# parsaeskandar/pangenome-index

Measured on AMD Instinct MI355X. Metric: find_mems reads/sec (150 bp batch), higher is better.
Workload: dtype u64

## Files before the change

### pangenome-index_amd/csrc/pgx_batch.hip

```cpp
#include <memory>
#include <string>
#include <thread>

#include "pgx_runtime_internal.hpp"

struct pgx_chunk { uint64_t r0, r1, slot_base, slots; };

struct pgx_batch {
    pgx_index *h = nullptr;
    pgx_device_image *dimg = nullptr;
    int device = 0;
    hipStream_t own = nullptr;
    hipStream_t side = nullptr;
    hipEvent_t ev_side[2] = {nullptr, nullptr};
    bool class_valid = false, class_ok = false;
    uint64_t side_reads_est = 0;
    uint64_t n_reads = 0, read_bytes = 0;
    HostBuf h_off[2];
    int h_off_cur = 0;
    const uint64_t *h_offsets() const { return h_off[h_off_cur].as<uint64_t>(); }
    std::vector<pgx_chunk> chunks;
    bool plan_valid = false, slot_off_valid = false;
    uint64_t slot_off_min_len = 0;
    uint64_t plan_min_len = 0, plan_budget = 0;
// ... 292 lines not shown
    PGX_GUARD_END
}

extern "C" pgx_status pgx_batch_upload_text(pgx_batch *b, const uint8_t *text, uint64_t n_bytes, uint32_t format, uint64_t *n_reads) {
    PGX_GUARD_BEGIN
    RoctxRange range("pgx_batch_upload_text");
    if (!b || !n_reads || (!text && n_bytes)) throw Error(PGX_ERR_ARG, "pgx_batch_upload_text: null argument");
    if (format > PGX_READS_FASTQ) throw Error(PGX_ERR_ARG, "pgx_batch_upload_text: unknown format " + std::to_string(format));
    use_device(b->device);
    batch_upload_text(b, text, n_bytes, format, n_reads);
    return PGX_OK;
    PGX_GUARD_END
}


struct RunKnobs {
    bool spec;
    bool arena;
    bool has_arena_cap;
    uint64_t arena_cap;
    uint64_t budget_slots;
    bool narrow;
    bool force_redo;
    bool pairs;
    bool side;
    bool packed;
    int coop;
    bool lce;
    bool has_wg_per_cu;
    int wg_per_cu;
    uint32_t heavy_ext;
    bool has_side_heavy_ext;
    uint32_t side_heavy_ext;
    bool debug_counters;
    bool fm_stats;
};

static RunKnobs read_run_knobs() {
    auto is_set = [](const char *name) { return std::getenv(name) != nullptr; };
    auto not_zero = [](const char *name) { const char *e = std::getenv(name); return !(e && e[0] == '0'); };
    RunKnobs k{};
    k.spec = not_zero("PGX_SPEC");
    k.arena = not_zero("PGX_SLOT_ARENA");
    if (const char *e = std::getenv("PGX_SLOT_ARENA_CAP")) { k.has_arena_cap = true; k.arena_cap = std::strtoull(e, nullptr, 10); }
    if (const char *e = std::getenv("PGX_SLOT_BUDGET_MB")) k.budget_slots = std::max<uint64_t>(1, std::strtoull(e, nullptr, 10)) * (1ull << 20) / sizeof(pgx_mem);
    k.narrow = not_zero("PGX_FM_NARROW");
    k.force_redo = is_set("PGX_FM_NARROW_FORCE_REDO");
    k.pairs = not_zero("PGX_FM_PAIRS");
    k.side = !is_set("PGX_FM_NO_SIDE");
    k.packed = not_zero("PGX_FM_PACKED");
    k.coop = -1;
    if (const char *e = std::getenv("PGX_FM_COOP")) k.coop = e[0] == '1';
    k.lce = not_zero("PGX_FM_LCE");
    if (const char *e = std::getenv("PGX_FM_WG_PER_CU")) { k.has_wg_per_cu = true; k.wg_per_cu = std::atoi(e); }
    k.heavy_ext = PGX_FM_HEAVY_EXT;
    if (const char *e = std::getenv("PGX_FM_HEAVY_EXT")) k.heavy_ext = (uint32_t)std::strtoul(e, nullptr, 10);
    if (const char *e = std::getenv("PGX_FM_SIDE_HEAVY_EXT")) { k.has_side_heavy_ext = true; k.side_heavy_ext = (uint32_t)std::strtoul(e, nullptr, 10); }
    k.debug_counters = is_set("PGX_DEBUG_COUNTERS");
    k.fm_stats = is_set("PGX_FM_STATS");
    return k;
}

static const void *find_mems_entry(bool in_lds, uint32_t kind, bool narrow, bool seeded) {
    using K = const void *;
    static const K tab[2][4][2][2] = {
        {{{(K)pgx_find_mems_kernel<false, 0, false, false>, nullptr}, {nullptr, nullptr}},
         {{(K)pgx_find_mems_kernel<false, 1, false, false>, (K)pgx_find_mems_kernel<false, 1, false, true>},
          {(K)pgx_find_mems_kernel<false, 1, true, false>, (K)pgx_find_mems_kernel<false, 1, true, true>}},
         {{(K)pgx_find_mems_kernel<false, 2, false, false>, (K)pgx_find_mems_kernel<false, 2, false, true>},
          {(K)pgx_find_mems_kernel<false, 2, true, false>, (K)pgx_find_mems_kernel<false, 2, true, true>}},
         {{(K)pgx_find_mems_kernel<false, 3, false, false>, (K)pgx_find_mems_kernel<false, 3, false, true>}, {nullptr, nullptr}}},
        {{{(K)pgx_find_mems_kernel<true, 0, false, false>, nullptr}, {nullptr, nullptr}},
         {{(K)pgx_find_mems_kernel<true, 1, false, false>, (K)pgx_find_mems_kernel<true, 1, false, true>},
          {(K)pgx_find_mems_kernel<true, 1, true, false>, (K)pgx_find_mems_kernel<true, 1, true, true>}},
         {{nullptr, nullptr}, {nullptr, nullptr}},
         {{nullptr, nullptr}, {nullptr, nullptr}}}};
    return kind < 4 ? tab[in_lds][kind][narrow][seeded] : nullptr;
}

static uint32_t find_mems_bits(bool in_lds, uint32_t kind, bool narrow, bool seeded) {
    return PGX_KERNELS_FM | (seeded ? PGX_KERNELS_FM_SEEDED : 0u) | (narrow ? PGX_KERNELS_FM_NARROW : 0u) | (kind << PGX_KERNELS_FM_KIND_SHIFT) | (in_lds ? PGX_KERNELS_FM_LDS : 0u);
}

static const void *find_mems_variant(bool in_lds, uint32_t kind, bool narrow, bool seeded, uint32_t &bits) {
    if (kind == 0) seeded = false;
    const void *f = find_mems_entry(in_lds, kind, narrow, seeded);
    if (!f) throw Error(PGX_ERR_UNSUPPORTED, "pgx_batch_run: no find_mems kernel for this image");
    bits = find_mems_bits(in_lds, kind, narrow, seeded);
    return f;
}
// ... 12 lines not shown
    if (lce) return (wide || !packed || coop) ? nullptr : with_lce[s64];
    if (!packed) return coop ? nullptr : plain[wide][s64];
    return pack[wide][coop][s64];
}

static uint32_t find_mems_pairs_bits(bool wide, bool packed, bool coop, bool s64, bool lce) {
    return PGX_KERNELS_PAIRS | (s64 ? PGX_KERNELS_PAIRS_S64 : 0u) | (coop ? PGX_KERNELS_PAIRS_COOP : 0u) | (packed ? PGX_KERNELS_PAIRS_PACKED : 0u) |
           (wide ? PGX_KERNELS_PAIRS_WIDE : 0u) | (lce ? PGX_KERNELS_PAIRS_LCE : 0u);
}

static const void *find_mems_pairs_variant(bool wide, bool packed, bool coop, bool s64, bool lce, uint32_t &bits) {
    const void *f = find_mems_pairs_entry(wide, packed, coop, s64, lce);
    if (!f && lce) throw Error(PGX_ERR_UNSUPPORTED, "pgx_batch_run: no LCE pairs kernel for this image");
    if (!f) throw Error(PGX_ERR_UNSUPPORTED, "pgx_batch_run: no cooperative pairs kernel without the packed reads");
    bits = find_mems_pairs_bits(wide, packed, coop, s64, lce);
    return f;
}

extern "C" uint32_t pgx_kernel_variants(uint32_t *out, uint32_t cap) {
    uint32_t n = 0;
    auto put = [&](uint32_t bits) { if (out && n < cap) out[n] = bits; n++; };
    for (int c = 0; c < 32; c++) {
        const bool in_lds = c & 16, narrow = c & 2, seeded = c & 1;
        const uint32_t kind = (c >> 2) & 3;
        if (find_mems_entry(in_lds, kind, narrow, seeded)) put(find_mems_bits(in_lds, kind, narrow, seeded));
    }
    for (int c = 0; c < 32; c++) {
        const bool wide = c & 16, packed = c & 8, coop = c & 4, s64 = c & 2, lce = c & 1;
        if (find_mems_pairs_entry(wide, packed, coop, s64, lce)) put(find_mems_pairs_bits(wide, packed, coop, s64, lce));
    }
    return n;
}

struct RunCtx {
    pgx_batch *b;
    hipStream_t s;
    RunKnobs k;
    PgxDevImage img;
    uint64_t n, min_len, min_occ;
    bool want_tags;
    unsigned long long *ctr = nullptr;
    bool spec = false, arena_on = false;
    uint64_t cm_cap = 0;
    const void *kfn = nullptr, *kfn_wide = nullptr, *kfn_pairs = nullptr;
    uint32_t kfn_bits = 0, kfn_pairs_bits = 0;
    size_t pairs_lds = 0;
    int cus = 0;
    bool fresh_work = false, fresh_mark = false;
    uint64_t n_ext = 0;
    float ms_fm = 0, ms_cp = 0, ms_main = 0;
};

struct FmArgs {
    PgxDevImage img;
    const uint8_t *reads;
    const uint64_t *off, *slot_off;
    uint64_t n, min_len, min_occ, base, first;
    pgx_mem *slots;
    uint32_t *cnt;
    unsigned long long *next, *cur;
    uint32_t hext, hcap;
    pgx_heavy_item *hlist;
    unsigned long long *hcount;
    uint32_t *ovf;
    uint64_t ovf_cap;
};

static void record(pgx_batch *b, int i, hipStream_t s) {
    static const char *const stage[10] = {"pgx: run begins (classify, sizing)", "pgx: find_mems launches follow", "pgx: find_mems enqueued", "pgx: compaction enqueued",
                                          "pgx: tag locate enqueued", "pgx: tag gather enqueued", "pgx: tag sort/unique enqueued", "pgx: run enqueued", "pgx: main find_mems kernel enqueued",
                                          "pgx: per-upload passes enqueued"};
    if (roctx().on) roctx().mark(stage[i]);
    if (!b->timed) return;
    if (!b->ev[i]) HIPCHECK(hipEventCreate(&b->ev[i]));
    HIPCHECK(hipEventRecord(b->ev[i], s));
}

static unsigned find_mems_grid(const RunCtx &r, const void *kfn, size_t lds, bool few_suffice, uint64_t cn) {
    int wg = 0;
    HIPCHECK(hipOccupancyMaxActiveBlocksPerMultiprocessor(&wg, kfn, PGX_FM_THREADS, lds));
// ... 62 lines not shown

static void classify_reads(RunCtx &r, uint64_t cn) {
    pgx_batch *b = r.b;
    hipStream_t s = r.s;
    r.fresh_work = true;
    const uint64_t cap = std::max<uint64_t>(cn, 1024);
    b->read_flags.ensure(((cn + 3) & ~3ull) + 4);
    b->side_list.ensure((cn ? cn : 1) * sizeof(pgx_heavy_item));
    b->side_count.ensure(16);
    b->scan_tmp.ensure(cap * 8);
    b->scan_tmp.scan_epoch = 0;
    b->packed.ensure(((b->read_bytes + 15) / 16 + 64) * 4);
    HIPCHECK(hipMemsetAsync(b->side_count.p, 0, 16, s));
    HIPCHECK(hipMemsetAsync(b->read_flags.p, 0, ((cn + 3) & ~3ull) + 4, s));
    unsigned long long *d_bad = b->side_count.as<unsigned long long>() + 1;
    hipLaunchKernelGGL(pgx_bad_chunks_kernel, dim3(std::min<unsigned>(grid_for((b->read_bytes + 15) / 16, 256), (unsigned)r.cus * 16u)), dim3(256), 0, s,
                       (const uint8_t *)b->reads.as<uint8_t>(), b->read_bytes, b->scan_tmp.as<uint64_t>(), d_bad, cap, b->packed.as<uint32_t>());
    HIPCHECK(hipGetLastError());
    unsigned long long n_bad = 0;
    read_scalars(&n_bad, d_bad, sizeof n_bad, s);
    b->class_ok = n_bad <= cap;
    b->side_reads_est = n_bad / 4;
    if (b->class_ok && n_bad) {
        hipLaunchKernelGGL(pgx_classify_reads_kernel, dim3(grid_for(n_bad, 256)), dim3(256), 0, s, (const uint8_t *)b->reads.as<uint8_t>(),
                           (const uint64_t *)b->offsets.as<uint64_t>(), cn, (const uint64_t *)b->scan_tmp.as<uint64_t>(), (const unsigned long long *)d_bad, cap,
                           b->read_flags.as<uint32_t>(), b->side_list.as<pgx_heavy_item>(), b->side_count.as<unsigned long long>());
        HIPCHECK(hipGetLastError());
    }
    b->class_valid = true;
}

static void launch_side(RunCtx &r, FmArgs &a, const void *kf, unsigned grid) {
    pgx_batch *b = r.b;
    HIPCHECK(hipEventRecord(b->ev_side[0], r.s));
    HIPCHECK(hipStreamWaitEvent(b->side, b->ev_side[0], 0));
    const pgx_heavy_item *s_list = b->side_list.as<pgx_heavy_item>();
    const unsigned long long *s_count = b->side_count.as<unsigned long long>();
    unsigned long long *s_cur = r.ctr + PGX_CTR_SIDE_CURSOR;
    uint32_t s_hext = r.k.heavy_ext ? std::min<uint32_t>(r.k.heavy_ext, PGX_FM_SIDE_HEAVY_EXT) : 0u;
    if (r.k.has_side_heavy_ext) s_hext = r.k.side_heavy_ext;
    void *sargs[] = {&a.img, &a.reads, &a.off, &a.n, &a.min_len, &a.min_occ, &a.slot_off, &a.slots, &a.cnt, &a.next, &s_cur, &a.first, &a.base,
                     &s_hext, &a.hcap, &a.hlist, &a.hcount, &s_list, &s_count, &a.ovf, &a.ovf_cap};
    const uint64_t cus = (uint64_t)r.cus;
    const unsigned side_wgs = (unsigned)std::min<uint64_t>(4 * cus, std::max<uint64_t>(cus, b->side_reads_est / (2ull * PGX_FM_THREADS) + 1));
    HIPCHECK(hipLaunchKernel(kf, dim3(std::min<unsigned>(grid, side_wgs)), dim3(PGX_FM_THREADS), sargs, b->dimg->lds_bytes, b->side));
    b->timing.kernels |= r.kfn_bits | PGX_KERNELS_SIDE | (kf != r.kfn ? PGX_KERNELS_FM_REDO : 0u);
    HIPCHECK(hipEventRecord(b->ev_side[1], b->side));
}

static void launch_pairs(RunCtx &r, FmArgs &a, const uint8_t *skip, uint64_t cn, unsigned grid) {
    pgx_batch *b = r.b;
    const PgxDevImage &img = r.img;
    const void *kp = r.kfn_pairs;
    uint32_t kp_bits = r.kfn_pairs_bits;
    size_t plds = r.pairs_lds;
    const uint32_t *a_packed = nullptr;
    uint32_t a_pkw = 0;
    const uint32_t pkw = (uint32_t)((15 + b->max_read_len + 15) >> 4) + 1u;
    if (skip && pkw <= 24 && r.k.packed) {
        const bool coop = r.k.coop >= 0 ? r.k.coop != 0 : b->h->img.pairs.size() > (3ull << 30);
        const bool lce = img.lce_sa && !coop && !img.wide && r.min_occ <= 1 && r.k.lce;
        kp = find_mems_pairs_variant(img.wide != 0, true, coop, img.pairs_stride == PGX_PAIRS_STRIDE64, lce, kp_bits);
        const size_t lce_lds = lce ? (size_t)PGX_FM_THREADS * (16 + 4 + 20) : 0;
        a_packed = b->packed.as<uint32_t>();
        a_pkw = pkw;
        plds = (size_t)pkw * PGX_FM_THREADS * 4 + (coop ? (size_t)(PGX_FM_THREADS / 64) * 8192 : 0) + (img.wide ? (size_t)img.n_sbp * 192 : 0) + lce_lds;
        b->timing.pairs_reads = lce ? 4u : coop ? 3u : 2u;
        grid = find_mems_grid(r, kp, plds, true, cn);
    }
    void *pargs[] = {&a.img, &a.reads, &a.off, &a.n, &a.min_len, &a.min_occ, &a.slot_off, &a.slots, &a.cnt, &a.next, &a.cur, &a.first, &a.base,
                     &a.hext, &a.hcap, &a.hlist, &a.hcount, &skip, &a_packed, &a_pkw, &a.ovf, &a.ovf_cap};
    HIPCHECK(hipLaunchKernel(kp, dim3(grid), dim3(PGX_FM_THREADS), pargs, plds, r.s));
    b->timing.kernels |= kp_bits;
}

static uint64_t arena_slots(const RunCtx &r, const pgx_chunk &c) {
    const pgx_batch *b = r.b;
    if (!r.arena_on) return 0;
    const uint64_t cn = c.r1 - c.r0;
    uint64_t want = b->shape_valid && b->shape_reads == r.n && b->shape_min_len == r.min_len && b->chunks.size() == 1 ? with_slack(b->last_ovf_used) + 4096 : 8 * cn + 4096;
    if (r.k.has_arena_cap) want = r.k.arena_cap;
    want = std::max<uint64_t>(want, b->max_read_len + 1);
    want = std::max<uint64_t>(want, (uint64_t)PGX_ARENA_SUBS * (b->max_read_len + 1));
    want = (want + PGX_ARENA_SUBS - 1) / PGX_ARENA_SUBS * PGX_ARENA_SUBS;
    return want < c.slots && want < (1ull << 32) ? want : 0;
}

static uint64_t find_mems_chunk(RunCtx &r, size_t ci, uint64_t &ovf_cap) {
    pgx_batch *b = r.b;
    hipStream_t s = r.s;
    const pgx_chunk &c = b->chunks[ci];
    const uint64_t cn = c.r1 - c.r0;
    const bool one_chunk = b->chunks.size() == 1;
    const uint32_t heavy_ext = r.k.heavy_ext;
    const unsigned grid = find_mems_grid(r, r.kfn_pairs ? r.kfn_pairs : r.kfn, r.kfn_pairs ? r.pairs_lds : b->dimg->lds_bytes, r.img.dense != 0, cn);
    uint64_t *local = b->mem_off.as<uint64_t>() + c.r0;
    const void *kf = r.kfn;
    ovf_cap = arena_slots(r, c);
    for (int attempt = 0;; attempt++) {
        b->slots.ensure(((ovf_cap ? ovf_cap : c.slots) + 4 * cn) * sizeof(pgx_mem));
        if (ci || attempt) {
            HIPCHECK(hipMemsetAsync(r.ctr, 0, PGX_CTR_TAG0 * 8, s));
            HIPCHECK(hipMemsetAsync(r.ctr + PGX_CTR_ARENA0, 0, (PGX_CTR_ALL - PGX_CTR_ARENA0) * 8, s));
        }
        FmArgs a;
        a.img = r.img;
        a.reads = b->reads.as<uint8_t>();
        a.off = b->offsets.as<uint64_t>(); a.slot_off = b->slot_off.as<uint64_t>();
        a.n = c.r1; a.min_len = r.min_len; a.min_occ = r.min_occ; a.base = c.slot_base; a.first = c.r0;
        a.slots = b->slots.as<pgx_mem>();
        a.cnt = b->mem_count.as<uint32_t>();
        a.next = r.ctr; a.cur = r.ctr + PGX_CTR_CURSOR;
        a.hext = heavy_ext; a.hcap = PGX_FM_HEAVY_CAP;
        a.hlist = b->heavy_list.as<pgx_heavy_item>();
        a.hcount = r.ctr + PGX_CTR_HEAVY;
        a.ovf = b->ovf_base.as<uint32_t>() - c.r0;
        a.ovf_cap = ovf_cap;
        bool side_running = false;
        if (r.kfn_pairs) {
            const uint8_t *skip = nullptr;
            if (one_chunk && r.k.side) {
                if (!b->side) {
                    HIPCHECK(hipStreamCreateWithFlags(&b->side, hipStreamNonBlocking));
                    for (auto &e : b->ev_side) HIPCHECK(hipEventCreateWithFlags(&e, hipEventDisableTiming));
                }
                if (!b->class_valid) classify_reads(r, cn);
                record(b, 9, s); r.fresh_mark = true;
                if (b->class_ok) {
                    skip = b->read_flags.as<uint8_t>();
                    launch_side(r, a, kf, grid);
                    side_running = true;
                }
            }
            launch_pairs(r, a, skip, cn, grid);
        } else {
            const pgx_heavy_item *a_rlist = nullptr;
            const unsigned long long *a_rcount = nullptr;
            void *args[] = {&a.img, &a.reads, &a.off, &a.n, &a.min_len, &a.min_occ, &a.slot_off, &a.slots, &a.cnt, &a.next, &a.cur, &a.first, &a.base,
                            &a.hext, &a.hcap, &a.hlist, &a.hcount, &a_rlist, &a_rcount, &a.ovf, &a.ovf_cap};
            if (ci == 0 && attempt == 0) { record(b, 9, s); r.fresh_mark = true; }
            HIPCHECK(hipLaunchKernel(kf, dim3(grid), dim3(PGX_FM_THREADS), args, b->dimg->lds_bytes, s));
            b->timing.kernels |= r.kfn_bits | (kf != r.kfn ? PGX_KERNELS_FM_REDO : 0u);
        }
        record(b, 8, s);
        if (side_running) HIPCHECK(hipStreamWaitEvent(s, b->ev_side[1], 0));
        if (heavy_ext) {
            b->timing.kernels |= PGX_KERNELS_HEAVY;
            if (b->dimg->lds_bytes)
                hipLaunchKernelGGL(pgx_find_mems_heavy_kernel<true>, dim3(PGX_FM_HEAVY_GRID), dim3(256), b->dimg->lds_bytes, s, r.img, a.reads, a.off,
                                   r.min_len, r.min_occ, a.slot_off, c.slot_base, a.slots, a.cnt, r.ctr, (const pgx_heavy_item *)a.hlist,
                                   (const unsigned long long *)a.hcount, (uint32_t)PGX_FM_HEAVY_CAP, b->heavy_scratch.as<PgxHeavyResult>(), c.r0, cn, a.ovf, a.ovf_cap);
            else
                hipLaunchKernelGGL(pgx_find_mems_heavy_kernel<false>, dim3(PGX_FM_HEAVY_GRID), dim3(256), 0, s, r.img, a.reads, a.off, r.min_len, r.min_occ,
                                   a.slot_off, c.slot_base, a.slots, a.cnt, r.ctr, (const pgx_heavy_item *)a.hlist,
                                   (const unsigned long long *)a.hcount, (uint32_t)PGX_FM_HEAVY_CAP, b->heavy_scratch.as<PgxHeavyResult>(), c.r0, cn, a.ovf, a.ovf_cap);
        }
        if (ovf_cap) hipLaunchKernelGGL(pgx_arena_demand_kernel, dim3(1), dim3(PGX_ARENA_SUBS), 0, s, r.ctr);
        HIPCHECK(hipGetLastError());
        b->timing.find_mems_launches++;
        record(b, 2, s);
        scan_excl(0, b->mem_count.as<uint32_t>() + c.r0, cn, 0, local, b->scan_tmp, s, reinterpret_cast<uint64_t *>(r.ctr + PGX_CTR_MEMS));
        if (r.spec) return r.cm_cap;
        unsigned long long cc[16];
        read_scalars(cc, r.ctr, sizeof cc, s);
        if (ovf_cap) b->last_ovf_used = cc[PGX_CTR_OVF_TOP];
        if (ovf_cap && cc[PGX_CTR_OVF_ABORT]) { ovf_cap = 0; continue; }
        const bool forced = attempt == 0 && kf != r.kfn_wide && r.k.force_redo;
        if ((cc[PGX_CTR_OVF32] || forced) && kf != r.kfn_wide) { kf = r.kfn_wide; continue; }
        r.n_ext += cc[PGX_CTR_EXT];
        b->timing.heavy_reads += (uint32_t)std::min<unsigned long long>(cc[PGX_CTR_HEAVY], PGX_FM_HEAVY_CAP);
        b->timing.pairs_other_steps += (uint32_t)cc[PGX_CTR_REDO];
        return cc[PGX_CTR_MEMS];
    }
}

static void compact_chunk(RunCtx &r, const pgx_chunk &c, uint64_t cm, uint64_t mem_base, uint64_t ovf_cap) {
    pgx_batch *b = r.b;
    hipStream_t s = r.s;
    const uint64_t cn = c.r1 - c.r0;
    b->mems.ensure_keep((mem_base + cm ? mem_base + cm : 1) * sizeof(pgx_mem), mem_base * sizeof(pgx_mem));
    hipLaunchKernelGGL(pgx_compact_mems_kernel, dim3(grid_for(cn, 256)), dim3(256), 0, s, c.r0, cn, b->slot_off.as<uint64_t>(),
                       c.slot_base, b->slots.as<pgx_mem>(), b->mem_count.as<uint32_t>(), (const uint64_t *)(b->mem_off.as<uint64_t>() + c.r0), mem_base,
                       b->mems.as<pgx_mem>(), r.spec ? r.cm_cap : ~0ull, reinterpret_cast<uint64_t *>(r.ctr + PGX_CTR_ABORT),
                       (const uint32_t *)(b->ovf_base.as<uint32_t>() - c.r0), ovf_cap);
    HIPCHECK(hipGetLastError());
    record(b, 3, s);
    if (b->timed && b->chunks.size() > 1) {
        HIPCHECK(hipStreamSynchronize(s));
// ... 62 lines not shown
        if (r.want_tags) {
            b->timing.ms_tag_locate = el(3, 4);
            b->timing.ms_tag_gather = el(4, 5);
            b->timing.ms_tag_sort = el(5, 6);
        }
        b->timing.ms_total = el(0, 7);
        if (r.fresh_work) b->timing.ms_per_upload = b->ms_upload_passes + (r.fresh_mark ? el(0, 9) : 0.0f);
    }
    if (r.fresh_work) b->ms_upload_passes = 0;
    return true;
}

static bool run_pass(RunCtx &r, bool may_speculate, bool &force_worst) {
    pgx_batch *b = r.b;
    hipStream_t s = r.s;
    b->n_mems = b->n_positions = b->n_ext = b->n_tag_overflow = 0;
    std::memset(&b->timing, 0, sizeof b->timing);
    r.fresh_work = r.fresh_mark = false;
    r.n_ext = 0;
    r.ms_fm = r.ms_cp = r.ms_main = 0;
    b->counters.ensure(PGX_CTR_ALL * 8);
    HIPCHECK(hipMemsetAsync(b->counters.p, 0, PGX_CTR_ALL * 8, s));
    r.ctr = b->counters.as<unsigned long long>();

    record(b, 0, s);
    plan_slots(r);
    const std::vector<pgx_chunk> &chunks = b->chunks;
    r.arena_on = r.k.arena && !force_worst;
    r.kfn = r.kfn_wide = r.kfn_pairs = nullptr;
    r.cus = 0;
    if (r.n) choose_kernels(r);
    if (r.k.heavy_ext) {
        b->heavy_list.ensure((size_t)PGX_FM_HEAVY_CAP * sizeof(pgx_heavy_item));
        b->heavy_scratch.ensure((size_t)PGX_FM_HEAVY_GRID * PGX_FM_HEAVY_MAXLEN * sizeof(PgxHeavyResult));
    }
    r.spec = may_speculate && chunks.size() == 1 && b->shape_valid && b->shape_reads == r.n && b->shape_min_len == r.min_len && b->shape_min_occ == r.min_occ &&
             b->shape_tags == r.want_tags && (!r.want_tags || (b->tw.have_last && b->tw.last_largest <= PGX_SORT_WG_LDS_CAP)) && r.k.spec && !r.k.force_redo;
    r.cm_cap = with_slack(b->last_mems);
    uint64_t mem_base = 0;
    for (size_t ci = 0; ci < chunks.size(); ci++) {
        record(b, 1, s);
        uint64_t ovf_cap = 0;
        const uint64_t cm = find_mems_chunk(r, ci, ovf_cap);
        compact_chunk(r, chunks[ci], cm, mem_base, ovf_cap);
        mem_base += cm;
    }
    b->n_mems = mem_base;
    if (!r.kfn_pairs) b->timing.pairs_reads = 0u;
    else if (!b->timing.pairs_reads) b->timing.pairs_reads = 1u;
    b->timing.seed_depth = (r.img.seed_k != 0 && r.min_len >= r.img.seed_k && r.img.dense) ? r.img.seed_k : 0u;
    if (chunks.size() != 1) {
        if (chunks.empty()) { record(b, 1, s); record(b, 2, s); }
        scan_excl(0, b->mem_count.p, r.n, 0, b->mem_off.as<uint64_t>(), b->scan_tmp, s);
        b->mems.ensure_keep((b->n_mems ? b->n_mems : 1) * sizeof(pgx_mem), b->n_mems * sizeof(pgx_mem));
        record(b, 3, s);
    }
    record(b, 3, s);
    if (r.want_tags) {
        tag_pipeline(r.img, b->mems.as<pgx_mem>(), nullptr, nullptr, b->n_mems, b->tw, r.ctr + PGX_CTR_TAG_OVERFLOW, r.ctr + PGX_CTR_TAG0, s,
                     [&](int stage) { record(b, 4 + stage, s); }, r.spec, reinterpret_cast<const uint64_t *>(r.ctr + PGX_CTR_MEMS),
                     reinterpret_cast<uint64_t *>(r.ctr + PGX_CTR_ABORT));
        b->n_positions = b->tw.n_positions;
        b->ran_tags = true;
    }
    record(b, 7, s);
    return read_back(r, force_worst);
}
// ... 379 lines not shown
```

### pangenome-index_amd/csrc/pgx_device.h

```cpp
#pragma once

#include <hip/hip_runtime.h>
#include <stdint.h>

#include "../../include/pgx.h"
#include "pgx_image.h"

enum PgxCounterSlot {
    PGX_CTR_EXT = 0,
    PGX_CTR_TAG_OVERFLOW = 1,
    PGX_CTR_CURSOR = 5,
    PGX_CTR_HEAVY = 8,
    PGX_CTR_OVF32 = 9,
    PGX_CTR_MEMS = 10,
    PGX_CTR_REDO = 11,
    PGX_CTR_REDO_CURSOR = 12,
    PGX_CTR_SIDE_CURSOR = 13,
    PGX_CTR_OVF_TOP = 14,
    PGX_CTR_OVF_ABORT = 15,
    PGX_CTR_TAG0 = 16,
    PGX_CTR_ABORT = 30,
    PGX_CTR_PAIRS_LINES = 32,
    PGX_CTR_PAIRS_SEEDS = 33,
    PGX_CTR_FM_LINES = 34,
// ... 43 lines not shown
    const uint4 *seed_main, *seed_small;
    const uint4 *pairs;
    const uint4 *first_ext;
    uint32_t pair_runs;
    const uint64_t *sbase2, *pbase;
    uint32_t d2_sb_shift, pairs_sb_shift, n_sb2, n_sbp;
    uint32_t wide;
    uint32_t pairs_stride;
    const uint32_t *lce_sa;
    const uint32_t *lce_text;
    const uint32_t *lce_flags;
    const uint8_t *lce_lcp;
    uint32_t lce_max;
    uint32_t refill_min;
};
#define PGX_LCP_CAP 254u
#define PGX_LCP_UNKNOWN 255u
#define PGX_SEED_UNUSABLE 255u
#define PGX_SEED_MAX_K 16
#define PGX_SEED_SMALL_K 10

struct pgx_heavy_item {
    uint64_t rid;
    uint32_t x, nm;
};
struct PgxHeavyResult {
    pgx_mem mem;
    uint32_t next_x, n_ext, has_mem, pad;
};
#define PGX_FM_HEAVY_EXT 2048u
#define PGX_FM_SIDE_HEAVY_EXT 2048u
#define PGX_FM_HEAVY_MAXLEN 4096u
#define PGX_FM_HEAVY_CAP 8192u
#define PGX_FM_HEAVY_GRID 64u

template <bool LDS_IMAGE, int DENSE, bool NARROW, bool SEED>
__global__ void pgx_find_mems_kernel(PgxDevImage img, const uint8_t *reads, const uint64_t *offsets, uint64_t n_reads,
                                     uint64_t min_len, uint64_t min_occ, const uint64_t *slot_off, pgx_mem *slots,
                                     uint32_t *mem_count, unsigned long long *n_ext_total, unsigned long long *cursor, uint64_t first_read,
                                     uint64_t slot_base, uint32_t heavy_ext, uint32_t heavy_cap, pgx_heavy_item *heavy_list, unsigned long long *heavy_count,
                                     const pgx_heavy_item *rid_list, const unsigned long long *rid_count, uint32_t *ovf_base, uint64_t ovf_cap);
template <bool LDS_IMAGE>
__global__ void pgx_find_mems_heavy_kernel(PgxDevImage img, const uint8_t *reads, const uint64_t *offsets, uint64_t min_len, uint64_t min_occ,
                                           const uint64_t *slot_off, uint64_t slot_base, pgx_mem *slots, uint32_t *mem_count,
                                           unsigned long long *n_ext_total, const pgx_heavy_item *heavy_list,
                                           const unsigned long long *heavy_count, uint32_t heavy_cap, PgxHeavyResult *scratch, uint64_t chunk_first,
                                           uint64_t chunk_reads, uint32_t *ovf_base, uint64_t ovf_cap);
__global__ void pgx_fmf_kernel(PgxDevImage img, const uint8_t *reads, const uint64_t *offsets, const uint64_t *read_of, const uint64_t *xs, uint64_t n,
                               uint64_t min_len, uint64_t min_occ, PgxHeavyResult *out);
__global__ void pgx_arena_demand_kernel(unsigned long long *ctr);

template <bool WIDE, bool PACKED, bool COOP, bool S64, bool LCE>
__global__ void pgx_find_mems_pairs_kernel(PgxDevImage img, const uint8_t *reads, const uint64_t *offsets, uint64_t n_reads,
                                           uint64_t min_len, uint64_t min_occ, const uint64_t *slot_off, pgx_mem *slots,
                                           uint32_t *mem_count, unsigned long long *n_ext_total, unsigned long long *cursor, uint64_t first_read,
                                           uint64_t slot_base, uint32_t heavy_ext, uint32_t heavy_cap, pgx_heavy_item *heavy_list, unsigned long long *heavy_count,
                                           const uint8_t *skip, const uint32_t *packed, uint32_t pk_words,
                                           uint32_t *ovf_base, uint64_t ovf_cap);

__global__ void pgx_bad_chunks_kernel(const uint8_t *reads, uint64_t n_bytes, uint64_t *chunks, unsigned long long *count, uint64_t cap, uint32_t *packed);
__global__ void pgx_unpack_reads_kernel(const uint32_t *packed, uint64_t n_chunks, uint8_t *reads);
__global__ void pgx_side_reads_kernel(uint8_t *reads, const uint64_t *offsets, const uint64_t *side_ids, const uint64_t *side_off, const uint8_t *side_bytes, uint64_t n_side,
                                      uint8_t *flags, pgx_heavy_item *list, unsigned long long *count);
__global__ void pgx_classify_reads_kernel(const uint8_t *reads, const uint64_t *offsets, uint64_t n_reads, const uint64_t *chunks, const unsigned long long *n_chunks,
                                          uint64_t cap, uint32_t *flag_words, pgx_heavy_item *list, unsigned long long *count);

__global__ void pgx_seed_build_kernel(PgxDevImage img, const uint4 *src, uint4 *dst, uint32_t level, uint64_t n_dst, uint64_t limit, int end_table);
__global__ void pgx_first_ext_kernel(PgxDevImage img, uint4 *out);
__global__ void pgx_rank_kernel(PgxDevImage img, const uint64_t *pos, uint64_t n, int true_codes, uint64_t *out);
template <bool LOOP, bool MULHI> __global__ void pgx_rank_probe_kernel(PgxDevImage img, const uint64_t *pos, uint64_t n, uint64_t *out);
template <bool LDS_IMAGE>
__global__ void pgx_extend_kernel(PgxDevImage img, const pgx_biint *in, const uint8_t *sym, const uint8_t *forward, uint64_t n,
                                  pgx_biint *out);
template <bool LDS_IMAGE>
__global__ void pgx_count_kernel(PgxDevImage img, const uint8_t *reads, const uint64_t *offsets, uint64_t n_reads, pgx_range *out);
__global__ void pgx_lf_kernel(PgxDevImage img, const pgx_range *in, const uint8_t *sym, uint64_t n, pgx_range *out);

__global__ void pgx_scan_partial_kernel(int mode, const void *in, uint64_t n, uint64_t min_len, uint64_t *block_sums, const uint64_t *n_dev);
template <int MODE>
// ... 136 lines not shown
```

### pangenome-index_amd/csrc/pgx_fm_kernels.hip

```cpp
#include <hip/hip_runtime.h>
#include <stdint.h>

#include <type_traits>

#include "pgx_device.h"
#include "pgx_rank_device.h"
#include "pgx_slots_device.h"

#define PGX_FM_BATCH (LDS_IMAGE ? 128u : 32u)
template <bool LDS_IMAGE, int DENSE, bool NARROW, bool SEED>
__global__ void __launch_bounds__(PGX_FM_THREADS, DENSE == 0 ? 3 : PGX_FM_WAVES_PER_SIMD)
pgx_find_mems_kernel(PgxDevImage img, const uint8_t *__restrict__ reads, const uint64_t *__restrict__ offsets,
                     uint64_t n_reads, uint64_t min_len, uint64_t min_occ, const uint64_t *__restrict__ slot_off,
                     pgx_mem *__restrict__ slots, uint32_t *__restrict__ mem_count, unsigned long long *__restrict__ n_ext_total,
                     unsigned long long *__restrict__ cursor, uint64_t first_read, uint64_t slot_base, uint32_t heavy_ext, uint32_t heavy_cap,
                     pgx_heavy_item *__restrict__ heavy_list, unsigned long long *__restrict__ heavy_count,
                     const pgx_heavy_item *__restrict__ rid_list, const unsigned long long *__restrict__ rid_count, uint32_t *__restrict__ ovf_base, uint64_t ovf_cap) {
    __shared__ uint32_t s_ext[512];
    __shared__ uint64_t s_C[8];
    __shared__ uint64_t s_sb[DENSE == 3 ? PGX_SB_MAX * 8 : 1];
    PGX_LDS_CARVE(img);
    if (DENSE == 3) for (uint32_t i = threadIdx.x; i < img.n_sb2 * 8u; i += blockDim.x) s_sb[i] = img.sbase2[i];
    pgx_stage_tables<LDS_IMAGE>(img, s_ext, s_C, lds_blocks, lds_dir, lds_blow);
    const uint64_t chunk_first = first_read, chunk_reads = n_reads - first_read;
// ... 319 lines not shown
            if (s < min_occ || s == 0) { r.next_x = (uint32_t)(j + 1); dead = true; break; }
        }
        if (!dead) {
            uint64_t Jk = k, Js = s;
            int32_t j = xs + (int32_t)min_len;
            for (; j < len; j++) {
                pgx_extend<LDS_IMAGE>(img, lds_blocks, lds_dir, lds_blow, s_ext, s_C, k, kp, s, pat[j], true);
                ne++;
                if (s < min_occ || s == 0) break;
                Jk = k; Js = s;
            }
            r.has_mem = 1;
            r.mem.end = (uint64_t)j; r.mem.bwt_start = Jk; r.mem.size = (int64_t)Js;
            k = 0; kp = 0; s = n;
            uint32_t nxt = (uint32_t)(xs + 1);
            for (; j > xs; j--) {
                pgx_extend<LDS_IMAGE>(img, lds_blocks, lds_dir, lds_blow, s_ext, s_C, k, kp, s, j < len ? pat[j] : (uint8_t)0, false);
                ne++;
                if (s < min_occ || s == 0) { nxt = (uint32_t)(j + 1); break; }
            }
            r.next_x = nxt;
        }
        r.n_ext = ne;
    }
    return r;
}

template <bool LDS_IMAGE>
__global__ void __launch_bounds__(256)
pgx_find_mems_heavy_kernel(PgxDevImage img, const uint8_t *__restrict__ reads, const uint64_t *__restrict__ offsets, uint64_t min_len,
                           uint64_t min_occ, const uint64_t *__restrict__ slot_off, uint64_t slot_base, pgx_mem *__restrict__ slots,
                           uint32_t *__restrict__ mem_count, unsigned long long *__restrict__ n_ext_total,
                           const pgx_heavy_item *__restrict__ heavy_list, const unsigned long long *__restrict__ heavy_count,
                           uint32_t heavy_cap, PgxHeavyResult *__restrict__ scratch, uint64_t chunk_first, uint64_t chunk_reads,
                           uint32_t *__restrict__ ovf_base, uint64_t ovf_cap) {
    unsigned long long cnt = *heavy_count;
    if (cnt == 0) return;
    if (cnt > heavy_cap) cnt = heavy_cap;
    __shared__ uint32_t s_ext[512];
    __shared__ uint64_t s_C[8];
    PGX_LDS_CARVE(img);
    pgx_stage_tables<LDS_IMAGE>(img, s_ext, s_C, lds_blocks, lds_dir, lds_blow);
    PgxHeavyResult *res = scratch + (size_t)blockIdx.x * PGX_FM_HEAVY_MAXLEN;
    for (unsigned long long h = blockIdx.x; h < cnt; h += gridDim.x) {
        const pgx_heavy_item it = heavy_list[h];
        const uint64_t base = offsets[it.rid];
        const int32_t len = (int32_t)(offsets[it.rid + 1] - base), x0 = (int32_t)it.x;
        const uint8_t *pat = reads + base;
        for (int32_t xs = x0 + (int32_t)threadIdx.x; xs < len; xs += (int32_t)blockDim.x) {
            const PgxHeavyResult r = pgx_fmf_eval<LDS_IMAGE>(img, lds_blocks, lds_dir, lds_blow, s_ext, s_C, pat, len, xs, min_len, min_occ);
            res[xs - x0] = r;
        }
        __threadfence_block();
        __syncthreads();
        if (threadIdx.x == 0) {
            uint32_t nm = it.nm;
            unsigned long long ne = 0;
            int32_t x = x0;
            while (x < len && (uint64_t)(len - x) >= min_len) {
                const PgxHeavyResult r = res[x - x0];
                ne += r.n_ext;
                if (r.has_mem) {
                    const uint64_t slot = nm < PGX_FAST_SLOTS ? 0ull : pgx_slot_extent(slot_off, slot_base, ovf_base, ovf_cap, n_ext_total, it.rid, nm, len, x, min_len);
                    slots[pgx_slot_index(it.rid - chunk_first, chunk_reads, slot, nm)] = r.mem; nm++;
                }
                x = (int32_t)r.next_x;
            }
            mem_count[it.rid] = nm;
            atomicAdd(n_ext_total, ne);
        }
        __syncthreads();
    }
}
template __global__ void pgx_find_mems_heavy_kernel<false>(PgxDevImage, const uint8_t *, const uint64_t *, uint64_t, uint64_t, const uint64_t *, uint64_t,
                                                           pgx_mem *, uint32_t *, unsigned long long *, const pgx_heavy_item *,
                                                           const unsigned long long *, uint32_t, PgxHeavyResult *, uint64_t, uint64_t, uint32_t *, uint64_t);
template __global__ void pgx_find_mems_heavy_kernel<true>(PgxDevImage, const uint8_t *, const uint64_t *, uint64_t, uint64_t, const uint64_t *, uint64_t,
                                                          pgx_mem *, uint32_t *, unsigned long long *, const pgx_heavy_item *,
                                                          const unsigned long long *, uint32_t, PgxHeavyResult *, uint64_t, uint64_t, uint32_t *, uint64_t);

__global__ void __launch_bounds__(256)
pgx_fmf_kernel(PgxDevImage img, const uint8_t *__restrict__ reads, const uint64_t *__restrict__ offsets, const uint64_t *__restrict__ read_of,
               const uint64_t *__restrict__ xs, uint64_t n, uint64_t min_len, uint64_t min_occ, PgxHeavyResult *__restrict__ out) {
    __shared__ uint32_t s_ext[512];
    __shared__ uint64_t s_C[8];
    pgx_stage_tables<false>(img, s_ext, s_C, nullptr, nullptr, nullptr);
    const uint64_t i = (uint64_t)blockIdx.x * blockDim.x + threadIdx.x;
    if (i >= n) return;
    const uint64_t rid = read_of[i], base = offsets[rid];
    const int32_t len = (int32_t)(offsets[rid + 1] - base);
    PgxHeavyResult r;
    if (xs[i] > (uint64_t)len) {
        r.mem.start = xs[i]; r.mem.end = 0; r.mem.bwt_start = 0; r.mem.size = 0;
        r.next_x = (uint32_t)len; r.n_ext = 0; r.has_mem = 0; r.pad = 0;
    } else {
        r = pgx_fmf_eval<false>(img, nullptr, nullptr, nullptr, s_ext, s_C, reads + base, len, (int32_t)xs[i], min_len, min_occ);
    }
    out[i] = r;
}
```

Measured before the change: 1.121 billion.

## Size heavy-read kernel launch from occupancy and read length, stage results in LDS

The heavy-read kernel used to launch with a fixed 64-block grid of 256 threads. It now takes its grid from occupancy times CU count, capped by a scratch budget, and its block size from the number of possible start positions in the longest read. For short remaining suffixes, per-start results go to a shared-memory buffer instead of global scratch, and blocks with no work exit early. An env flag can also run the side kernel on the main stream. The aim is better GPU fill for the heavy tail and less global scratch traffic, at the cost of more LDS per block and an occupancy query on the host each run.

After: 1.120 billion. About the same (-0.1%).

```diff
diff --git a/pangenome-index_amd/csrc/pgx_batch.hip b/pangenome-index_amd/csrc/pgx_batch.hip
--- a/pangenome-index_amd/csrc/pgx_batch.hip
+++ b/pangenome-index_amd/csrc/pgx_batch.hip
@@ -348,6 +348,7 @@
     uint32_t heavy_ext;
     bool has_side_heavy_ext;
     uint32_t side_heavy_ext;
+    bool side_serial;
     bool debug_counters;
     bool fm_stats;
 };
@@ -372,6 +373,7 @@
     k.heavy_ext = PGX_FM_HEAVY_EXT;
     if (const char *e = std::getenv("PGX_FM_HEAVY_EXT")) k.heavy_ext = (uint32_t)std::strtoul(e, nullptr, 10);
     if (const char *e = std::getenv("PGX_FM_SIDE_HEAVY_EXT")) { k.has_side_heavy_ext = true; k.side_heavy_ext = (uint32_t)std::strtoul(e, nullptr, 10); }
+    if (const char *e = std::getenv("PGX_FM_SIDE_SERIAL")) k.side_serial = e[0] != '0';
     k.debug_counters = is_set("PGX_DEBUG_COUNTERS");
     k.fm_stats = is_set("PGX_FM_STATS");
     return k;
@@ -450,6 +452,10 @@
     return n;
 }
 
+struct HeavyShape {
+    unsigned grid = 1, block = 64;
+    uint32_t stride = 1;
+};
 struct RunCtx {
     pgx_batch *b;
     hipStream_t s;
@@ -464,6 +470,7 @@
     uint32_t kfn_bits = 0, kfn_pairs_bits = 0;
     size_t pairs_lds = 0;
     int cus = 0;
+    HeavyShape heavy = {};
     bool fresh_work = false, fresh_mark = false;
     uint64_t n_ext = 0;
     float ms_fm = 0, ms_cp = 0, ms_main = 0;
@@ -592,8 +599,12 @@
 
 static void launch_side(RunCtx &r, FmArgs &a, const void *kf, unsigned grid) {
     pgx_batch *b = r.b;
-    HIPCHECK(hipEventRecord(b->ev_side[0], r.s));
-    HIPCHECK(hipStreamWaitEvent(b->side, b->ev_side[0], 0));
+    const bool serial = r.k.side_serial;
+    hipStream_t st = serial ? r.s : b->side;
+    if (!serial) {
+        HIPCHECK(hipEventRecord(b->ev_side[0], r.s));
+        HIPCHECK(hipStreamWaitEvent(b->side, b->ev_side[0], 0));
+    }
     const pgx_heavy_item *s_list = b->side_list.as<pgx_heavy_item>();
     const unsigned long long *s_count = b->side_count.as<unsigned long long>();
     unsigned long long *s_cur = r.ctr + PGX_CTR_SIDE_CURSOR;
@@ -603,9 +614,9 @@
                      &s_hext, &a.hcap, &a.hlist, &a.hcount, &s_list, &s_count, &a.ovf, &a.ovf_cap};
     const uint64_t cus = (uint64_t)r.cus;
     const unsigned side_wgs = (unsigned)std::min<uint64_t>(4 * cus, std::max<uint64_t>(cus, b->side_reads_est / (2ull * PGX_FM_THREADS) + 1));
-    HIPCHECK(hipLaunchKernel(kf, dim3(std::min<unsigned>(grid, side_wgs)), dim3(PGX_FM_THREADS), sargs, b->dimg->lds_bytes, b->side));
+    HIPCHECK(hipLaunchKernel(kf, dim3(std::min<unsigned>(grid, side_wgs)), dim3(PGX_FM_THREADS), sargs, b->dimg->lds_bytes, st));
     b->timing.kernels |= r.kfn_bits | PGX_KERNELS_SIDE | (kf != r.kfn ? PGX_KERNELS_FM_REDO : 0u);
-    HIPCHECK(hipEventRecord(b->ev_side[1], b->side));
+    if (!serial) HIPCHECK(hipEventRecord(b->ev_side[1], b->side));
 }
 
 static void launch_pairs(RunCtx &r, FmArgs &a, const uint8_t *skip, uint64_t cn, unsigned grid) {
@@ -632,6 +643,20 @@
                      &a.hext, &a.hcap, &a.hlist, &a.hcount, &skip, &a_packed, &a_pkw, &a.ovf, &a.ovf_cap};
     HIPCHECK(hipLaunchKernel(kp, dim3(grid), dim3(PGX_FM_THREADS), pargs, plds, r.s));
     b->timing.kernels |= kp_bits;
+}
+
+static HeavyShape heavy_launch_shape(const RunCtx &r) {
+    const pgx_batch *b = r.b;
+    HeavyShape h;
+    h.stride = (uint32_t)std::max<uint64_t>(1, std::min<uint64_t>(b->max_read_len, PGX_FM_HEAVY_MAXLEN));
+    const uint64_t starts = (uint64_t)h.stride >= r.min_len ? (uint64_t)h.stride - r.min_len + 1 : 1;
+    h.block = (unsigned)std::min<uint64_t>(256, (starts + 63) / 64 * 64);
+    int wg = 0;
+    const void *kh = b->dimg->lds_bytes ? (const void *)pgx_find_mems_heavy_kernel<true> : (const void *)pgx_find_mems_heavy_kernel<false>;
+    HIPCHECK(hipOccupancyMaxActiveBlocksPerMultiprocessor(&wg, kh, (int)h.block, b->dimg->lds_bytes));
+    const uint64_t by_scratch = (uint64_t)PGX_FM_HEAVY_SCRATCH_MAX / ((uint64_t)h.stride * sizeof(PgxHeavyResult));
+    h.grid = (unsigned)std::max<uint64_t>(1, std::min<uint64_t>(std::min<uint64_t>((uint64_t)std::max(wg, 1) * (uint64_t)r.cus, PGX_FM_HEAVY_CAP), by_scratch));
+    return h;
 }
 
 static uint64_t arena_slots(const RunCtx &r, const pgx_chunk &c) {
@@ -689,7 +714,7 @@
                 if (b->class_ok) {
                     skip = b->read_flags.as<uint8_t>();
                     launch_side(r, a, kf, grid);
-                    side_running = true;
+                    side_running = !r.k.side_serial;
                 }
             }
             launch_pairs(r, a, skip, cn, grid);
@@ -706,14 +731,15 @@
         if (side_running) HIPCHECK(hipStreamWaitEvent(s, b->ev_side[1], 0));
         if (heavy_ext) {
             b->timing.kernels |= PGX_KERNELS_HEAVY;
+            const HeavyShape &hs = r.heavy;
             if (b->dimg->lds_bytes)
-                hipLaunchKernelGGL(pgx_find_mems_heavy_kernel<true>, dim3(PGX_FM_HEAVY_GRID), dim3(256), b->dimg->lds_bytes, s, r.img, a.reads, a.off,
+                hipLaunchKernelGGL(pgx_find_mems_heavy_kernel<true>, dim3(hs.grid), dim3(hs.block), b->dimg->lds_bytes, s, r.img, a.reads, a.off,
                                    r.min_len, r.min_occ, a.slot_off, c.slot_base, a.slots, a.cnt, r.ctr, (const pgx_heavy_item *)a.hlist,
-                                   (const unsigned long long *)a.hcount, (uint32_t)PGX_FM_HEAVY_CAP, b->heavy_scratch.as<PgxHeavyResult>(), c.r0, cn, a.ovf, a.ovf_cap);
+                                   (const unsigned long long *)a.hcount, (uint32_t)PGX_FM_HEAVY_CAP, b->heavy_scratch.as<PgxHeavyResult>(), hs.stride, c.r0, cn, a.ovf, a.ovf_cap);
             else
-                hipLaunchKernelGGL(pgx_find_mems_heavy_kernel<false>, dim3(PGX_FM_HEAVY_GRID), dim3(256), 0, s, r.img, a.reads, a.off, r.min_len, r.min_occ,
+                hipLaunchKernelGGL(pgx_find_mems_heavy_kernel<false>, dim3(hs.grid), dim3(hs.block), 0, s, r.img, a.reads, a.off, r.min_len, r.min_occ,
                                    a.slot_off, c.slot_base, a.slots, a.cnt, r.ctr, (const pgx_heavy_item *)a.hlist,
-                                   (const unsigned long long *)a.hcount, (uint32_t)PGX_FM_HEAVY_CAP, b->heavy_scratch.as<PgxHeavyResult>(), c.r0, cn, a.ovf, a.ovf_cap);
+                                   (const unsigned long long *)a.hcount, (uint32_t)PGX_FM_HEAVY_CAP, b->heavy_scratch.as<PgxHeavyResult>(), hs.stride, c.r0, cn, a.ovf, a.ovf_cap);
         }
         if (ovf_cap) hipLaunchKernelGGL(pgx_arena_demand_kernel, dim3(1), dim3(PGX_ARENA_SUBS), 0, s, r.ctr);
         HIPCHECK(hipGetLastError());
@@ -842,7 +868,8 @@
     if (r.n) choose_kernels(r);
     if (r.k.heavy_ext) {
         b->heavy_list.ensure((size_t)PGX_FM_HEAVY_CAP * sizeof(pgx_heavy_item));
-        b->heavy_scratch.ensure((size_t)PGX_FM_HEAVY_GRID * PGX_FM_HEAVY_MAXLEN * sizeof(PgxHeavyResult));
+        if (r.n) r.heavy = heavy_launch_shape(r);
+        b->heavy_scratch.ensure((size_t)r.heavy.grid * r.heavy.stride * sizeof(PgxHeavyResult));
     }
     r.spec = may_speculate && chunks.size() == 1 && b->shape_valid && b->shape_reads == r.n && b->shape_min_len == r.min_len && b->shape_min_occ == r.min_occ &&
              b->shape_tags == r.want_tags && (!r.want_tags || (b->tw.have_last && b->tw.last_largest <= PGX_SORT_WG_LDS_CAP)) && r.k.spec && !r.k.force_redo;
diff --git a/pangenome-index_amd/csrc/pgx_device.h b/pangenome-index_amd/csrc/pgx_device.h
--- a/pangenome-index_amd/csrc/pgx_device.h
+++ b/pangenome-index_amd/csrc/pgx_device.h
@@ -99,7 +99,8 @@
 #define PGX_FM_SIDE_HEAVY_EXT 2048u
 #define PGX_FM_HEAVY_MAXLEN 4096u
 #define PGX_FM_HEAVY_CAP 8192u
-#define PGX_FM_HEAVY_GRID 64u
+#define PGX_FM_HEAVY_LDS_STARTS 256u
+#define PGX_FM_HEAVY_SCRATCH_MAX (64u << 20)
 
 template <bool LDS_IMAGE, int DENSE, bool NARROW, bool SEED>
 __global__ void pgx_find_mems_kernel(PgxDevImage img, const uint8_t *reads, const uint64_t *offsets, uint64_t n_reads,
@@ -111,7 +112,7 @@
 __global__ void pgx_find_mems_heavy_kernel(PgxDevImage img, const uint8_t *reads, const uint64_t *offsets, uint64_t min_len, uint64_t min_occ,
                                            const uint64_t *slot_off, uint64_t slot_base, pgx_mem *slots, uint32_t *mem_count,
                                            unsigned long long *n_ext_total, const pgx_heavy_item *heavy_list,
-                                           const unsigned long long *heavy_count, uint32_t heavy_cap, PgxHeavyResult *scratch, uint64_t chunk_first,
+                                           const unsigned long long *heavy_count, uint32_t heavy_cap, PgxHeavyResult *scratch, uint32_t stride, uint64_t chunk_first,
                                            uint64_t chunk_reads, uint32_t *ovf_base, uint64_t ovf_cap);
 __global__ void pgx_fmf_kernel(PgxDevImage img, const uint8_t *reads, const uint64_t *offsets, const uint64_t *read_of, const uint64_t *xs, uint64_t n,
                                uint64_t min_len, uint64_t min_occ, PgxHeavyResult *out);
diff --git a/pangenome-index_amd/csrc/pgx_fm_kernels.hip b/pangenome-index_amd/csrc/pgx_fm_kernels.hip
--- a/pangenome-index_amd/csrc/pgx_fm_kernels.hip
+++ b/pangenome-index_amd/csrc/pgx_fm_kernels.hip
@@ -375,21 +375,22 @@
                            uint64_t min_occ, const uint64_t *__restrict__ slot_off, uint64_t slot_base, pgx_mem *__restrict__ slots,
                            uint32_t *__restrict__ mem_count, unsigned long long *__restrict__ n_ext_total,
                            const pgx_heavy_item *__restrict__ heavy_list, const unsigned long long *__restrict__ heavy_count,
-                           uint32_t heavy_cap, PgxHeavyResult *__restrict__ scratch, uint64_t chunk_first, uint64_t chunk_reads,
+                           uint32_t heavy_cap, PgxHeavyResult *__restrict__ scratch, uint32_t stride, uint64_t chunk_first, uint64_t chunk_reads,
                            uint32_t *__restrict__ ovf_base, uint64_t ovf_cap) {
     unsigned long long cnt = *heavy_count;
-    if (cnt == 0) return;
     if (cnt > heavy_cap) cnt = heavy_cap;
+    if (blockIdx.x >= cnt) return;
     __shared__ uint32_t s_ext[512];
     __shared__ uint64_t s_C[8];
+    __shared__ PgxHeavyResult s_res[PGX_FM_HEAVY_LDS_STARTS];
     PGX_LDS_CARVE(img);
     pgx_stage_tables<LDS_IMAGE>(img, s_ext, s_C, lds_blocks, lds_dir, lds_blow);
-    PgxHeavyResult *res = scratch + (size_t)blockIdx.x * PGX_FM_HEAVY_MAXLEN;
     for (unsigned long long h = blockIdx.x; h < cnt; h += gridDim.x) {
         const pgx_heavy_item it = heavy_list[h];
         const uint64_t base = offsets[it.rid];
         const int32_t len = (int32_t)(offsets[it.rid + 1] - base), x0 = (int32_t)it.x;
         const uint8_t *pat = reads + base;
+        PgxHeavyResult *res = len - x0 <= (int32_t)PGX_FM_HEAVY_LDS_STARTS ? s_res : scratch + (size_t)blockIdx.x * stride;
         for (int32_t xs = x0 + (int32_t)threadIdx.x; xs < len; xs += (int32_t)blockDim.x) {
             const PgxHeavyResult r = pgx_fmf_eval<LDS_IMAGE>(img, lds_blocks, lds_dir, lds_blow, s_ext, s_C, pat, len, xs, min_len, min_occ);
             res[xs - x0] = r;
@@ -417,10 +418,10 @@
 }
 template __global__ void pgx_find_mems_heavy_kernel<false>(PgxDevImage, const uint8_t *, const uint64_t *, uint64_t, uint64_t, const uint64_t *, uint64_t,
                                                            pgx_mem *, uint32_t *, unsigned long long *, const pgx_heavy_item *,
-                                                           const unsigned long long *, uint32_t, PgxHeavyResult *, uint64_t, uint64_t, uint32_t *, uint64_t);
+                                                           const unsigned long long *, uint32_t, PgxHeavyResult *, uint32_t, uint64_t, uint64_t, uint32_t *, uint64_t);
 template __global__ void pgx_find_mems_heavy_kernel<true>(PgxDevImage, const uint8_t *, const uint64_t *, uint64_t, uint64_t, const uint64_t *, uint64_t,
                                                           pgx_mem *, uint32_t *, unsigned long long *, const pgx_heavy_item *,
-                                                          const unsigned long long *, uint32_t, PgxHeavyResult *, uint64_t, uint64_t, uint32_t *, uint64_t);
+                                                          const unsigned long long *, uint32_t, PgxHeavyResult *, uint32_t, uint64_t, uint64_t, uint32_t *, uint64_t);
 
 __global__ void __launch_bounds__(256)
 pgx_fmf_kernel(PgxDevImage img, const uint8_t *__restrict__ reads, const uint64_t *__restrict__ offsets, const uint64_t *__restrict__ read_of,
```
